# cxy1997/3D_adapt_auto_driving

Hardware: AMD Instinct MI355X
Metric: KITTI scenes/s end-to-end eval_rcnn (joint RPN+RCNN, synthetic 16384-pt scenes) (higher is better)
Workload: dtype f32; 1 GPU; BASELINE.json configs[2]: full PointRCNN RPN+RCNN inference, default.yaml shapes, random-init weights, batch=8 synthetic KITTI scenes x 16384 pts per GPU per step; scene=synth.scenes (SURVEY 8d: uniform clutter + ground + 10 dense cars), parallelism=scene-sharded x1, one final all_gather of detections, detections_gathered=652455, batch_slots=14, look_ahead=12, steps_per_launch=2

## Files before the change

3d_adapt_auto_driving_amd/csrc/fps.hip:

```cpp
#include "common.hpp"
#include <math.h>
#include <stdlib.h>
#include <map>
#include <mutex>

namespace prcnn {

__device__ __forceinline__ bool better(float v, uint32_t key, float bv, uint32_t bkey)
{
    return (v > bv) | ((v == bv) & (key < bkey));
}

__device__ __forceinline__ void take_if_better(float v, uint32_t key, float &bv, uint32_t &bkey)
{
    const bool t = better(v, key, bv, bkey);
    bv = t ? v : bv;
    bkey = t ? key : bkey;
}

template <int CTRL>
__device__ __forceinline__ int dpp_mov(int x)
{
    return __builtin_amdgcn_update_dpp(x, x, CTRL, 0xf, 0xf, false);
}
// ... 42 lines not shown
    else r = fmax_raw(v, __int_as_float(dpp_mov<CTRL>(__float_as_int(v))));
    return r;
}
template <int CTRL>
__device__ __forceinline__ uint32_t dpp_min(uint32_t v)
{
    uint32_t r;
    if constexpr (CTRL == 0xB1) PRCNN_DPP_OP("v_min_u32_dpp", uint32_t, "quad_perm:[1,0,3,2]");
    else if constexpr (CTRL == 0x4E) PRCNN_DPP_OP("v_min_u32_dpp", uint32_t, "quad_perm:[2,3,0,1]");
    else if constexpr (CTRL == 0x141) PRCNN_DPP_OP("v_min_u32_dpp", uint32_t, "row_half_mirror");
    else if constexpr (CTRL == 0x140) PRCNN_DPP_OP("v_min_u32_dpp", uint32_t, "row_mirror");
    else {
        const uint32_t o = (uint32_t)dpp_mov<CTRL>((int)v);
        r = o < v ? o : v;
    }
    return r;
}
__device__ __forceinline__ float wave_max_f32(float v)
{
    v = dpp_max<0xB1>(v); v = dpp_max<0x4E>(v); v = dpp_max<0x141>(v); v = dpp_max<0x140>(v);
    const float r0 = __int_as_float(__builtin_amdgcn_readlane(__float_as_int(v), 0));
    const float r1 = __int_as_float(__builtin_amdgcn_readlane(__float_as_int(v), 16));
    const float r2 = __int_as_float(__builtin_amdgcn_readlane(__float_as_int(v), 32));
    const float r3 = __int_as_float(__builtin_amdgcn_readlane(__float_as_int(v), 48));
    return fmaxf(fmaxf(r0, r1), fmaxf(r2, r3));
}
__device__ __forceinline__ uint32_t wave_min_u32(uint32_t v)
{
    v = dpp_min<0xB1>(v); v = dpp_min<0x4E>(v); v = dpp_min<0x141>(v); v = dpp_min<0x140>(v);
    const uint32_t r0 = (uint32_t)__builtin_amdgcn_readlane((int)v, 0), r1 = (uint32_t)__builtin_amdgcn_readlane((int)v, 16);
    const uint32_t r2 = (uint32_t)__builtin_amdgcn_readlane((int)v, 32), r3 = (uint32_t)__builtin_amdgcn_readlane((int)v, 48);
    const uint32_t a = r0 < r1 ? r0 : r1, b = r2 < r3 ? r2 : r3;
    return a < b ? a : b;
}
__device__ __forceinline__ unsigned long long pack_candidate(float v, uint32_t key)
{
    const uint32_t b = (uint32_t)__float_as_int(v);
    const uint32_t mono = (b & 0x80000000u) ? ~b : (b | 0x80000000u);
    return ((unsigned long long)mono << 32) | (unsigned long long)(~key);
}
__device__ __forceinline__ void unpack_candidate(unsigned long long w, float &v, uint32_t &key)
{
    const uint32_t mono = (uint32_t)(w >> 32);
    const uint32_t b = (mono & 0x80000000u) ? (mono & 0x7fffffffu) : ~mono;
    v = __int_as_float((int)b);
    key = ~(uint32_t)w;
}

template <bool HIPCC>
__device__ __forceinline__ float fps_dist(float px, float py, float pz, float ox, float oy, float oz)
{
    if (!HIPCC) return sqdist3(px, py, pz, ox, oy, oz);
    const float dx = px - ox, dy = py - oy, dz = pz - oz;
    return __fadd_rn(__fmaf_rn(dy, dy, __fmul_rn(dx, dx)), __fmul_rn(dz, dz));
}

struct KeyCodec {
    int log2bs;
    int sh;
    int hipcc;
    __device__ __forceinline__ uint32_t encode(int k) const
    {
        const uint32_t low = (uint32_t)k & ((1u << log2bs) - 1u);
        const uint32_t rev = log2bs ? (__brev(low) >> (32 - log2bs)) : 0u;
        return (rev << sh) | ((uint32_t)k >> log2bs);
    }
    __device__ __forceinline__ int decode(uint32_t key) const
    {
        const uint32_t hi = key >> sh;
        const uint32_t rev = log2bs ? (__brev(hi) >> (32 - log2bs)) : 0u;
        return (int)(((key & ((1u << sh) - 1u)) << log2bs) | rev);
    }
};

template <int WAVES, int PPT, bool ORDERED>
__global__ __launch_bounds__(64 * WAVES) void fps_reg_kernel(
    int n, int m, KeyCodec kc, const float *__restrict__ xyz, float *__restrict__ temp,
    int *__restrict__ idx, float *__restrict__ new_xyz = nullptr, const int *__restrict__ rejected = nullptr)
{
    constexpr int T = 64 * WAVES;
    __shared__ unsigned long long s_best[3];
    const int b = blockIdx.x;
    if (rejected && rejected[b] == 0) return;
    const float *__restrict__ cloud = xyz + (long)b * n * 3;
    float *__restrict__ mind = temp ? temp + (long)b * n : nullptr;
    int *__restrict__ sel = idx + (long)b * m;
    float *__restrict__ nxyz = new_xyz ? new_xyz + (long)b * m * 3 : nullptr;
    const int t = threadIdx.x;
    __builtin_amdgcn_s_setprio(3);

    float px[PPT], py[PPT], pz[PPT], pt[PPT];
    uint32_t pk[PPT];
#pragma unroll
    for (int i = 0; i < PPT; ++i) {
        const int k = t + i * T;
        if (k < n) {
            px[i] = cloud[3 * k]; py[i] = cloud[3 * k + 1]; pz[i] = cloud[3 * k + 2];
            pt[i] = mind ? mind[k] : 1e10f;
            pk[i] = kc.encode(k);
        } else {
            px[i] = py[i] = pz[i] = 0.f;
            pt[i] = -INFINITY;
            pk[i] = 0xffffffffu;
        }
    }
    if (WAVES > 1 && t < 3) s_best[t] = 0ull;
    if (WAVES > 1) __syncthreads();

    int old = 0;
    if (t == 0) sel[0] = 0;
    for (int j = 1; j < m; ++j) {
        float ox, oy, oz;
        if constexpr (WAVES == 1) {
            const int pl = old & 63, pi = old >> 6;
            ox = oy = oz = 0.f;
#pragma unroll
            for (int i = 0; i < PPT; ++i) {
                const float vx = __int_as_float(__builtin_amdgcn_readlane(__float_as_int(px[i]), pl));
                const float vy = __int_as_float(__builtin_amdgcn_readlane(__float_as_int(py[i]), pl));
                const float vz = __int_as_float(__builtin_amdgcn_readlane(__float_as_int(pz[i]), pl));
                if (i == pi) { ox = vx; oy = vy; oz = vz; }
            }
        } else {
            ox = cloud[3 * old]; oy = cloud[3 * old + 1]; oz = cloud[3 * old + 2];
        }
        if (nxyz && t == 0) { nxyz[3 * (j - 1)] = ox; nxyz[3 * (j - 1) + 1] = oy; nxyz[3 * (j - 1) + 2] = oz; }
        float lv = -INFINITY;
        if (kc.hipcc) {
#pragma unroll
            for (int i = 0; i < PPT; ++i) {
                const float d2 = fminf(fps_dist<true>(px[i], py[i], pz[i], ox, oy, oz), pt[i]);
                pt[i] = d2;
                lv = fmaxf(lv, d2);
            }
        } else {
#pragma unroll
            for (int i = 0; i < PPT; ++i) {
                const float d = sqdist3(px[i], py[i], pz[i], ox, oy, oz);
                const float d2 = fminf(d, pt[i]);
                pt[i] = d2;
                lv = fmaxf(lv, d2);
            }
        }
        float bv = wave_max_f32(lv);
        uint32_t lk = 0xffffffffu;
#pragma unroll
        for (int i = 0; i < PPT; ++i) {
            const uint32_t c = pt[i] == bv ? pk[i] : 0xffffffffu;
            lk = c < lk ? c : lk;
        }
        uint32_t bkey = wave_min_u32(lk);
        if (WAVES > 1) {
            const int buf = j % 3;
            if ((t & 63) == 0) atomicMax(&s_best[buf], pack_candidate(bv, bkey));
            lds_barrier();
            const unsigned long long best = s_best[buf];
            if (t == 0) s_best[(j + 2) % 3] = 0ull;
            unpack_candidate(best, bv, bkey);
        }
        old = (bkey == 0xffffffffu || !(bv > -1.0f)) ? 0 : kc.decode(bkey);
        old = __builtin_amdgcn_readfirstlane(old);
        if (t == 0) sel[j] = old;
        if (bv == 0.f) {
            for (int jj = j + 1 + t; jj < m; jj += T) {
                sel[jj] = 0;
                if (nxyz) { nxyz[3 * (jj - 1)] = cloud[0]; nxyz[3 * (jj - 1) + 1] = cloud[1]; nxyz[3 * (jj - 1) + 2] = cloud[2]; }
            }
            if (nxyz && t == 0) { nxyz[3 * j] = cloud[0]; nxyz[3 * j + 1] = cloud[1]; nxyz[3 * j + 2] = cloud[2]; }
            break;
        }
    }
    if (nxyz && t == 0 && m > 0) { nxyz[3 * (m - 1)] = cloud[3 * old]; nxyz[3 * (m - 1) + 1] = cloud[3 * old + 1]; nxyz[3 * (m - 1) + 2] = cloud[3 * old + 2]; }
    if (mind) {
#pragma unroll
        for (int i = 0; i < PPT; ++i) {
            const int k = t + i * T;
            if (k < n) mind[k] = pt[i];
        }
    }
}


__device__ __forceinline__ unsigned part1by1(unsigned v)
{
    v &= 0xffffu;
    v = (v | (v << 8)) & 0x00ff00ffu;
    v = (v | (v << 4)) & 0x0f0f0f0fu;
    v = (v | (v << 2)) & 0x33333333u;
    v = (v | (v << 1)) & 0x55555555u;
    return v;
}

__global__ __launch_bounds__(1024) void fps_order_kernel(int n, const float *__restrict__ xyz, int *__restrict__ perm,
                                                         const int *__restrict__ rejected = nullptr)
// ... 79 lines not shown
    if (rejected && rejected[b] == 0) return;
    const float *__restrict__ cloud = xyz + (long)b * n * 3;
    const int *__restrict__ order = perm + (long)b * n;
    float *__restrict__ mind = temp ? temp + (long)b * n : nullptr;
    int *__restrict__ sel = idx + (long)b * m;
    float *__restrict__ nxyz = new_xyz ? new_xyz + (long)b * m * 3 : nullptr;
    const int t = threadIdx.x, lane = t & 63, w = t >> 6;
    __builtin_amdgcn_s_setprio(3);

    float px[PPT], py[PPT], pz[PPT], pt[PPT];
    uint32_t pc[PPT];
    float bx0 = INFINITY, bx1 = -INFINITY, by0 = INFINITY, by1 = -INFINITY, bz0 = INFINITY, bz1 = -INFINITY;
#pragma unroll
    for (int i = 0; i < PPT; ++i) {
        const int s = w * (64 * PPT) + i * 64 + lane;
        float x0 = INFINITY, x1 = -INFINITY, y0 = INFINITY, y1 = -INFINITY, z0 = INFINITY, z1 = -INFINITY;
        if (s < n) {
            const int k = order[s];
            px[i] = cloud[3 * k]; py[i] = cloud[3 * k + 1]; pz[i] = cloud[3 * k + 2];
            pt[i] = mind ? mind[k] : 1e10f;
            pc[i] = (kc.encode(k) << SB) | (uint32_t)i;
            x0 = x1 = px[i]; y0 = y1 = py[i]; z0 = z1 = pz[i];
        } else {
            px[i] = py[i] = pz[i] = 0.f;
            pt[i] = -INFINITY;
            pc[i] = 0xffffffffu;
        }
#pragma unroll
        for (int d = 32; d >= 1; d >>= 1) {
            x0 = fmin_raw(x0, __shfl_xor(x0, d, 64)); x1 = fmax_raw(x1, __shfl_xor(x1, d, 64));
            y0 = fmin_raw(y0, __shfl_xor(y0, d, 64)); y1 = fmax_raw(y1, __shfl_xor(y1, d, 64));
            z0 = fmin_raw(z0, __shfl_xor(z0, d, 64)); z1 = fmax_raw(z1, __shfl_xor(z1, d, 64));
        }
        if (lane == i) { bx0 = x0; bx1 = x1; by0 = y0; by1 = y1; bz0 = z0; bz1 = z1; }
    }

    constexpr int GP = 64 / PPT;
    bx0 = __shfl(bx0, lane & (PPT - 1), 64); bx1 = __shfl(bx1, lane & (PPT - 1), 64);
    by0 = __shfl(by0, lane & (PPT - 1), 64); by1 = __shfl(by1, lane & (PPT - 1), 64);
    bz0 = __shfl(bz0, lane & (PPT - 1), 64); bz1 = __shfl(bz1, lane & (PPT - 1), 64);
    unsigned long long touched = 0ull, etiles = ~0ull;
    float bound = INFINITY;
    auto box_mask = [&](float ox, float oy, float oz, bool live) __attribute__((always_inline)) {
        const float dx = fmax_raw(fmax_raw(bx0 - ox, ox - bx1), 0.f);
        const float dy = fmax_raw(fmax_raw(by0 - oy, oy - by1), 0.f);
        const float dz = fmax_raw(fmax_raw(bz0 - oz, oz - bz1), 0.f);
        const float lb = dx * dx + dy * dy + dz * dz;
        return __ballot(live && !(lb * 0.99999f >= bound));
    };
    auto update = [&](float ox, float oy, float oz, unsigned long long mask) __attribute__((always_inline)) {
        if (mask != 0ull) {
            touched |= mask & etiles;
            const pk_f32x2 o_x = {ox, ox}, o_y = {oy, oy}, o_z = {oz, oz};
            if (kc.hipcc) {
#pragma unroll
                for (int i = 0; i < PPT; i += 2)
                    if ((mask >> i) & 3ull) {
                        const pk_f32x2 dx = (pk_f32x2){px[i], px[i + 1]} - o_x, dy = (pk_f32x2){py[i], py[i + 1]} - o_y,
                                       dz = (pk_f32x2){pz[i], pz[i + 1]} - o_z;
                        const pk_f32x2 d = __builtin_elementwise_fma(dy, dy, dx * dx) + dz * dz;
                        pt[i] = fmin_raw(d.x, pt[i]); pt[i + 1] = fmin_raw(d.y, pt[i + 1]);
                    }
            } else {
#pragma unroll
                for (int i = 0; i < PPT; i += 2)
                    if ((mask >> i) & 3ull) {
                        const pk_f32x2 dx = (pk_f32x2){px[i], px[i + 1]} - o_x, dy = (pk_f32x2){py[i], py[i + 1]} - o_y,
                                       dz = (pk_f32x2){pz[i], pz[i + 1]} - o_z;
                        const pk_f32x2 d = (dx * dx + dy * dy) + dz * dz;
                        pt[i] = fmin_raw(d.x, pt[i]); pt[i + 1] = fmin_raw(d.y, pt[i + 1]);
                    }
            }
        }
    };
    if (t == 0) {
        sel[0] = 0;
        if (nxyz) { nxyz[0] = cloud[0]; nxyz[1] = cloud[1]; nxyz[2] = cloud[2]; }
    }
    if (t < 32) { s_rank[t] = 0; s_blk[t] = 0; }
    int j = 1;
    if (m > 1) {
        const float ox = cloud[0], oy = cloud[1], oz = cloud[2];
        update(ox, oy, oz, box_mask(ox, oy, oz, lane < PPT));
    }
    touched = ~0ull;
    while (j < m) {
        if (touched != 0ull) {
            float bv = -INFINITY, sv = -INFINITY;
#pragma unroll
            for (int i = 0; i < PPT; ++i) {
                sv = __builtin_amdgcn_fmed3f(bv, sv, pt[i]);
                bv = fmax_raw(bv, pt[i]);
            }
            uint32_t lk = 0xffffffffu;
#pragma unroll
            for (int i = 0; i < PPT; ++i) {
                const uint32_t c = pt[i] == bv ? pc[i] : 0xffffffffu;
                lk = c < lk ? c : lk;
            }
            const float v1 = wave_max_f32(bv);
            const uint32_t c1 = wave_min_u32(bv == v1 ? lk : 0xffffffffu);
            const unsigned long long m1 = __ballot(bv == v1 && lk == c1);
            const int l1 = m1 ? (int)__builtin_ctzll(m1) : 0;
            const float bv2 = lane == l1 ? -INFINITY : bv;
            const float v2 = wave_max_f32(bv2);
            const uint32_t c2 = wave_min_u32(bv2 == v2 ? lk : 0xffffffffu);
            const unsigned long long m2 = __ballot(lane != l1 && bv2 == v2 && lk == c2);
            const int l2 = m2 ? (int)__builtin_ctzll(m2) : l1;
            const float v3 = wave_max_f32((lane == l1 || lane == l2) ? -INFINITY : bv);
            const float s1 = __int_as_float(__builtin_amdgcn_readlane(__float_as_int(sv), l1));
            const float s2 = __int_as_float(__builtin_amdgcn_readlane(__float_as_int(sv), l2));
            const float wB = fmax_raw(v3, fmax_raw(s1, s2));
            bound = v1;
            const int sl1 = (int)(c1 & ((1u << SB) - 1u)), sl2 = (int)(c2 & ((1u << SB) - 1u));
            const bool has2 = m2 != 0ull && c2 != 0xffffffffu;
            etiles = (1ull << sl1) | (has2 ? (1ull << sl2) : 0ull);
            float x1 = 0.f, y1 = 0.f, z1 = 0.f, x2 = 0.f, y2 = 0.f, z2 = 0.f;
            fs_pick3<PPT>(px, py, pz, __builtin_amdgcn_readfirstlane(sl1), l1, x1, y1, z1);
            fs_pick3<PPT>(px, py, pz, __builtin_amdgcn_readfirstlane(sl2), l2, x2, y2, z2);
            const float ex = lane == 0 ? x1 : x2, ey = lane == 0 ? y1 : y2, ez = lane == 0 ? z1 : z2;
            if (lane < 2) {
                const float ev = lane == 0 ? v1 : (has2 ? v2 : -INFINITY);
                const uint32_t ek = lane == 0 ? (c1 == 0xffffffffu ? 0xffffffffu : (c1 >> SB)) : (has2 ? (c2 >> SB) : 0xffffffffu);
                s_vk[2 * w + lane] = pack_candidate(ev, ek);
                s_xyz[2 * w + lane][0] = ex; s_xyz[2 * w + lane][1] = ey; s_xyz[2 * w + lane][2] = ez;
                if (lane == 0) s_bound[w] = wB;
            }
        }
        lds_barrier();
        const int left = m - j;
        const int e = lane & 31, h = lane >> 5;
        const unsigned long long pke = s_vk[e];
        float cv; uint32_t ck;
        unpack_candidate(pke, cv, ck);
        const float cx = s_xyz[e][0], cy = s_xyz[e][1], cz = s_xyz[e][2];
        const float gB = wave_max_f32(lane < 16 ? s_bound[lane] : -INFINITY);
        {
            const int i = 2 * w + h;
            const unsigned long long pki = s_vk[i];
            float iv; uint32_t ik;
            unpack_candidate(pki, iv, ik);
            const float ix = s_xyz[i][0], iy = s_xyz[i][1], iz = s_xyz[i][2];
            const bool before = pke > pki;
            const float d = kc.hipcc ? fps_dist<true>(ix, iy, iz, cx, cy, cz) : sqdist3(ix, iy, iz, cx, cy, cz);
            const unsigned long long bb = __ballot(before), kb = __ballot(before && (d < iv));
            if (e == 0) {
                s_rank[i] = __popc((unsigned)(h ? (bb >> 32) : bb));
                s_blk[i] = (unsigned)(h ? (kb >> 32) : kb) != 0u;
            }
        }
        lds_barrier();
        const int rank = s_rank[e];
        const bool blocked = s_blk[e] != 0;
        const bool valid = !(ck == 0xffffffffu || !(cv > -1.0f));
        const bool pass = rank == 0 ? true : ((cv > gB) && (cv > 0.f) && valid && !blocked);
        const bool stop = !pass || (rank == 0 && !valid);
        int r = (int)wave_min_u32((stop && !(rank == 0)) ? (uint32_t)rank : ((rank == 0 && !valid) ? 1u : 32u));
        r = min(min(r, left), FS_RMAX);
        if (r < 1) r = 1;
        const float ox_ = valid ? cx : cloud[0], oy_ = valid ? cy : cloud[1], oz_ = valid ? cz : cloud[2];
        if (w == 0 && h == 0 && rank < r) {
            sel[j + rank] = valid ? kc.decode(ck) : 0;
            if (nxyz) { nxyz[3 * (j + rank)] = ox_; nxyz[3 * (j + rank) + 1] = oy_; nxyz[3 * (j + rank) + 2] = oz_; }
        }
        const int dst = (h == 0 && rank < FS_RMAX) ? 3 * rank : 63;
        const float rv = __int_as_float(__builtin_amdgcn_ds_permute(dst << 2, __float_as_int(ox_)) |
                                        __builtin_amdgcn_ds_permute(min(dst + 1, 63) << 2, __float_as_int(oy_)) |
                                        __builtin_amdgcn_ds_permute(min(dst + 2, 63) << 2, __float_as_int(oz_)));
        j += r;
        const int apply_n = j >= m ? r - 1 : r;
        touched = 0ull;
        for (int q0 = 0; q0 < apply_n; q0 += GP) {
            const int qg = q0 + lane / PPT;
            const int src = 3 * min(qg, FS_RMAX - 1);
            const float gx = __shfl(rv, src, 64), gy = __shfl(rv, src + 1, 64), gz = __shfl(rv, src + 2, 64);
            const unsigned long long masks = box_mask(gx, gy, gz, qg < apply_n);
            if (masks == 0ull) continue;
#pragma unroll
            for (int g = 0; g < GP; ++g) {
                const unsigned long long mk = (masks >> (g * PPT)) & ((PPT == 64) ? ~0ull : ((1ull << PPT) - 1ull));
                if (mk != 0ull) {
                    const int q = q0 + g;
                    const float ox = __int_as_float(__builtin_amdgcn_readlane(__float_as_int(rv), 3 * q));
                    const float oy = __int_as_float(__builtin_amdgcn_readlane(__float_as_int(rv), 3 * q + 1));
                    const float oz = __int_as_float(__builtin_amdgcn_readlane(__float_as_int(rv), 3 * q + 2));
                    update(ox, oy, oz, mk);
                }
            }
        }
    }
    if (mind) {
#pragma unroll
        for (int i = 0; i < PPT; ++i)
            if (pc[i] != 0xffffffffu) mind[kc.decode(pc[i] >> SB)] = pt[i];
    }
}

struct Fps2Table {
    unsigned long long vk[2][64];
    float xyz[2][64][4];
    float bound[2][32];
    unsigned int sync;
    unsigned int pad[63];
};

__device__ __forceinline__ unsigned long long ld_agent_u64(const unsigned long long *p)
{
    return __hip_atomic_load(p, __ATOMIC_RELAXED, __HIP_MEMORY_SCOPE_AGENT);
}
__device__ __forceinline__ float ld_agent_f32(const float *p)
{
    return __int_as_float(__hip_atomic_load(reinterpret_cast<const int *>(p), __ATOMIC_RELAXED, __HIP_MEMORY_SCOPE_AGENT));
}

__device__ __forceinline__ void st_agent_u64(unsigned long long *p, unsigned long long v)
{
    __hip_atomic_store(p, v, __ATOMIC_RELAXED, __HIP_MEMORY_SCOPE_AGENT);
}
__device__ __forceinline__ void st_agent_f32(float *p, float v)
{
    __hip_atomic_store(reinterpret_cast<int *>(p), __float_as_int(v), __ATOMIC_RELAXED, __HIP_MEMORY_SCOPE_AGENT);
}

__global__ __launch_bounds__(1024) void fps_spec2_kernel(
    int nclouds, int n, int m, KeyCodec kc, const float *__restrict__ xyz, const int *__restrict__ perm,
    float *__restrict__ temp, int *__restrict__ idx, float *__restrict__ new_xyz, Fps2Table *__restrict__ tables)
{
    constexpr int PPT = 16, SB = 4, NE = 64;
    __shared__ unsigned long long s_vk[NE];
    __shared__ float s_xyz[NE][3];
    __shared__ float s_bound[32];
    __shared__ float s_res[64];
    __shared__ int s_rank[NE], s_blk[NE];
    __shared__ unsigned long long s_evk[32];
    __shared__ float s_exyz[32][3], s_eb[16];
    const int q_ = blockIdx.x;
    const int b = (q_ >> 4) * 8 + (q_ & 7), half = (q_ >> 3) & 1;
    if (b >= nclouds) return;
    const float *__restrict__ cloud = xyz + (long)b * n * 3;
    const int *__restrict__ order = perm + (long)b * n;
    float *__restrict__ mind = temp ? temp + (long)b * n : nullptr;
    int *__restrict__ sel = idx + (long)b * m;
    float *__restrict__ nxyz = new_xyz ? new_xyz + (long)b * m * 3 : nullptr;
    Fps2Table *__restrict__ tb = tables + b;
    const int t = threadIdx.x, lane = t & 63, w = t >> 6, gw = 16 * half + w;
    __builtin_amdgcn_s_setprio(3);

    float px[PPT], py[PPT], pz[PPT], pt[PPT];
    uint32_t pc[PPT];
    float bx0 = INFINITY, bx1 = -INFINITY, by0 = INFINITY, by1 = -INFINITY, bz0 = INFINITY, bz1 = -INFINITY;
#pragma unroll
// ... 414 lines not shown
    else if (n <= 16384) launch_reg<16, 16>(b, n, m, kc, xyz, temp, idx, st, nullptr, rejected);
    else hipLaunchKernelGGL(fps_generic_kernel, dim3(b), dim3(1024), 0, st, n, m, kc, xyz, temp, idx);
    return check_launch("furthest_point_sampling");
}

extern "C" int prcnn_furthest_point_sampling(int b, int n, int m, const float *xyz, float *temp,
                                             int *idx, void *stream)
{
    PRCNN_REQUIRE(temp || b == 0 || m == 0, "fps: null pointer");
    return fps_any(b, n, m, xyz, temp, idx, nullptr, stream);
}

static int fps_new_xyz_any(int b, int n, int m, const float *xyz, int *idx, float *new_xyz, void *stream, const int *rejected)
{
    if (n > 1024) return fps_any(b, n, m, xyz, nullptr, idx, new_xyz, stream, rejected);
    hipStream_t st = (hipStream_t)stream;
    KeyCodec kc;
    if (const int rc = fps_codec(n, &kc)) return rc;
    if (n <= 128) launch_reg<1, 2>(b, n, m, kc, xyz, nullptr, idx, st, new_xyz, rejected);
    else if (n <= 256) launch_reg<1, 4>(b, n, m, kc, xyz, nullptr, idx, st, new_xyz, rejected);
    else if (n <= 512) launch_reg<1, 8>(b, n, m, kc, xyz, nullptr, idx, st, new_xyz, rejected);
    else if (b >= 128) launch_reg<1, 16>(b, n, m, kc, xyz, nullptr, idx, st, new_xyz, rejected);
    else launch_reg<4, 4>(b, n, m, kc, xyz, nullptr, idx, st, new_xyz, rejected);
    return check_launch("fps_new_xyz");
}

extern "C" int prcnn_fps_new_xyz(int b, int n, int m, const float *xyz, int *idx, float *new_xyz, void *stream)
{
    PRCNN_REQUIRE(b >= 0 && n > 0 && m >= 0, "fps_new_xyz: b=%d n=%d m=%d", b, n, m);
    if (b == 0 || m == 0) return PRCNN_OK;
    PRCNN_REQUIRE(xyz && idx && new_xyz, "fps_new_xyz: null pointer");
    return fps_new_xyz_any(b, n, m, xyz, idx, new_xyz, stream, nullptr);
}

namespace prcnn {
constexpr int FPX_T = 256;

template <bool HIPCC>
__global__ __launch_bounds__(FPX_T) void fps_prefix_pivots_kernel(int n, int m, const float *__restrict__ xyz, float *__restrict__ dpiv,
                                                                  int *__restrict__ rejected, int *__restrict__ idx, float *__restrict__ new_xyz)
{
    __shared__ float s_p[FPX_T][3];
    __shared__ float s_part[4][64];
    const int b = blockIdx.y, t = threadIdx.x, lane = t & 63, w = t >> 6;
    const float *__restrict__ cloud = xyz + (long)b * n * 3;
    if (blockIdx.x == 0 && t == 0) rejected[b] = 0;
    const int s = blockIdx.x * 64 + lane;
    const int sc = min(s, m - 1);
    const float x = cloud[3 * sc], y = cloud[3 * sc + 1], z = cloud[3 * sc + 2];
    const int iend = min(blockIdx.x * 64 + 63, m - 1);
    float d = 1e10f;
    for (int i0 = 0; i0 < iend; i0 += FPX_T) {
        __syncthreads();
        if (i0 + t < iend) { s_p[t][0] = cloud[3 * (i0 + t)]; s_p[t][1] = cloud[3 * (i0 + t) + 1]; s_p[t][2] = cloud[3 * (i0 + t) + 2]; }
        __syncthreads();
        const int k1 = min(64, iend - i0 - 64 * w);
#pragma unroll 4
        for (int k = 0; k < k1; ++k) {
            const int q = 64 * w + k;
            const float e = fps_dist<HIPCC>(x, y, z, s_p[q][0], s_p[q][1], s_p[q][2]);
            d = (i0 + q < s) ? fminf(e, d) : d;
        }
    }
    s_part[w][lane] = d;
    __syncthreads();
    if (w == 0 && s < m) {
        dpiv[(long)b * m + s] = fminf(fminf(s_part[0][lane], s_part[1][lane]), fminf(s_part[2][lane], s_part[3][lane]));
        if (idx) idx[(long)b * m + s] = s;
        if (new_xyz) { float *o = new_xyz + ((long)b * m + s) * 3; o[0] = x; o[1] = y; o[2] = z; }
    }
}

template <bool HIPCC>
__global__ __launch_bounds__(FPX_T) void fps_prefix_check_kernel(int n, int m, KeyCodec kc, const float *__restrict__ xyz,
                                                                 const float *__restrict__ dpiv, int *__restrict__ rejected)
{
    __shared__ float4 s_p[FPX_T];
    const int b = blockIdx.y, t = threadIdx.x;
    const float *__restrict__ cloud = xyz + (long)b * n * 3;
    const float *__restrict__ D = dpiv + (long)b * m;
    const int j = blockIdx.x * FPX_T + t, jc = min(j, n - 1);
    const float x = cloud[3 * jc], y = cloud[3 * jc + 1], z = cloud[3 * jc + 2];
    const uint32_t kj = kc.encode(jc);
    bool ok = fabsf(x) < INFINITY && fabsf(y) < INFINITY && fabsf(z) < INFINITY;
    if (jc >= 1 && jc < m) ok &= D[jc] > 0.f;
    const int jmax = min(n, (int)(blockIdx.x + 1) * FPX_T) - 1;
    const int iend = min(m, jmax) - 1;
    float r = 1e10f;
    for (int i0 = 0; ; i0 += FPX_T) {
        const int seen = __hip_atomic_load(rejected + b, __ATOMIC_RELAXED, __HIP_MEMORY_SCOPE_AGENT);
        if (__syncthreads_or(!ok || seen != 0) || i0 >= iend) break;
        if (i0 + t < iend) {
            const int i = i0 + t;
            s_p[t] = make_float4(cloud[3 * i], cloud[3 * i + 1], cloud[3 * i + 2], D[i + 1]);
        }
        __syncthreads();
        const int k1 = min(FPX_T, iend - i0);
#pragma unroll 4
        for (int k = 0; k < k1; ++k) {
            const float4 p = s_p[k];
            const int s = i0 + k + 1;
            r = fminf(fps_dist<HIPCC>(x, y, z, p.x, p.y, p.z), r);
            bool win = p.w > r;
            if (p.w == r) win = kc.encode(s) < kj;
            ok = ok && (win || s >= jc);
        }
    }
    if (!ok) rejected[b] = 1;
}
}

extern "C" int prcnn_fps_nested_supported(int n, int m) { return m >= 2 && m <= n && n <= 16384; }

static int fps_prefix_any(int b, int n, int m, const KeyCodec &kc, const float *xyz, int *idx, float *new_xyz, float *dpiv, int *rejected,
                          hipStream_t st)
{
    const dim3 g1((unsigned)((m + 63) / 64), (unsigned)b), g2((unsigned)((n + FPX_T - 1) / FPX_T), (unsigned)b);
    if (kc.hipcc) {
        hipLaunchKernelGGL(fps_prefix_pivots_kernel<true>, g1, dim3(FPX_T), 0, st, n, m, xyz, dpiv, rejected, idx, new_xyz);
        hipLaunchKernelGGL(fps_prefix_check_kernel<true>, g2, dim3(FPX_T), 0, st, n, m, kc, xyz, dpiv, rejected);
    } else {
        hipLaunchKernelGGL(fps_prefix_pivots_kernel<false>, g1, dim3(FPX_T), 0, st, n, m, xyz, dpiv, rejected, idx, new_xyz);
        hipLaunchKernelGGL(fps_prefix_check_kernel<false>, g2, dim3(FPX_T), 0, st, n, m, kc, xyz, dpiv, rejected);
    }
    return check_launch("fps_prefix_check");
}

extern "C" int prcnn_fps_prefix_check(int b, int n, int m, const float *xyz, int *idx, float *new_xyz, int *rejected, void *stream)
{
    PRCNN_REQUIRE(b >= 0 && b <= 65535 && prcnn_fps_nested_supported(n, m), "fps_prefix_check: b=%d n=%d m=%d", b, n, m);
    if (b == 0) return PRCNN_OK;
    PRCNN_REQUIRE(xyz && rejected, "fps_prefix_check: null pointer");
    hipStream_t st = (hipStream_t)stream;
    KeyCodec kc;
    if (const int rc = fps_codec(n, &kc)) return rc;
    float *dpiv = (float *)scratch_for(st, (size_t)b * m * sizeof(float), 15);
    if (!dpiv) { set_error("fps_prefix_check: cannot allocate the pivot scratch"); return PRCNN_ELAUNCH; }
    return fps_prefix_any(b, n, m, kc, xyz, idx, new_xyz, dpiv, rejected, st);
}

extern "C" int prcnn_fps_new_xyz_flagged(int b, int n, int m, const float *xyz, int *idx, float *new_xyz, const int *rejected, void *stream)
{
    PRCNN_REQUIRE(b >= 0 && prcnn_fps_nested_supported(n, m), "fps_new_xyz_flagged: b=%d n=%d m=%d", b, n, m);
    if (b == 0) return PRCNN_OK;
    PRCNN_REQUIRE(xyz && idx && new_xyz && rejected, "fps_new_xyz_flagged: null pointer");
    return fps_new_xyz_any(b, n, m, xyz, idx, new_xyz, stream, rejected);
}

extern "C" int prcnn_fps_new_xyz_nested(int b, int n, int m, const float *xyz, int *idx, float *new_xyz, void *stream)
{
    PRCNN_REQUIRE(b >= 0 && n > 0 && m >= 0, "fps_new_xyz_nested: b=%d n=%d m=%d", b, n, m);
    if (b == 0 || m == 0) return PRCNN_OK;
    PRCNN_REQUIRE(xyz && idx && new_xyz, "fps_new_xyz_nested: null pointer");
    if (!prcnn_fps_nested_supported(n, m) || b > 65535) return fps_new_xyz_any(b, n, m, xyz, idx, new_xyz, stream, nullptr);
    hipStream_t st = (hipStream_t)stream;
    KeyCodec kc;
    if (const int rc = fps_codec(n, &kc)) return rc;
    float *dpiv = (float *)scratch_for(st, ((size_t)b * m + (size_t)b) * sizeof(float), 15);
    if (!dpiv) { set_error("fps_new_xyz_nested: cannot allocate the check's scratch"); return PRCNN_ELAUNCH; }
    int *rejected = (int *)(dpiv + (size_t)b * m);
    if (const int rc = fps_prefix_any(b, n, m, kc, xyz, idx, new_xyz, dpiv, rejected, st)) return rc;
    return fps_new_xyz_any(b, n, m, xyz, idx, new_xyz, stream, rejected);
}
namespace prcnn {
__global__ __launch_bounds__(256) void point_groups_kernel(int n, const float *__restrict__ xyz, const int *__restrict__ perm,
                                                           float4 *__restrict__ pxyz, float4 *__restrict__ aabb)
{
    const int b = blockIdx.y, lane = threadIdx.x & 63;
    const int g = blockIdx.x * 4 + (threadIdx.x >> 6);
    if (g * 64 >= n) return;
    const long s = (long)b * n + g * 64 + lane;
    const int k = perm[s];
    const float *p = xyz + ((long)b * n + k) * 3;
    const float x = p[0], y = p[1], z = p[2];
    pxyz[s] = make_float4(x, y, z, __int_as_float(k));
    float x0 = x, x1 = x, y0 = y, y1 = y, z0 = z, z1 = z;
#pragma unroll
    for (int d = 32; d >= 1; d >>= 1) {
        x0 = fminf(x0, __shfl_xor(x0, d, 64)); x1 = fmaxf(x1, __shfl_xor(x1, d, 64));
        y0 = fminf(y0, __shfl_xor(y0, d, 64)); y1 = fmaxf(y1, __shfl_xor(y1, d, 64));
        z0 = fminf(z0, __shfl_xor(z0, d, 64)); z1 = fmaxf(z1, __shfl_xor(z1, d, 64));
    }
    if (lane == 0) {
        aabb[((long)b * (n / 64) + g) * 2] = make_float4(x0, y0, z0, 0.f);
        aabb[((long)b * (n / 64) + g) * 2 + 1] = make_float4(x1, y1, z1, 0.f);
    }
}
}

extern "C" int prcnn_point_groups(int b, int n, const float *xyz, float *pxyz, float *aabb, void *stream)
{
    PRCNN_REQUIRE(b >= 0 && n > 0 && n % 64 == 0 && n <= 65536 && b <= 65535, "point_groups: b=%d n=%d (n a multiple of 64, <= 65536)", b, n);
    if (b == 0) return PRCNN_OK;
    PRCNN_REQUIRE(xyz && pxyz && aabb && (((uintptr_t)pxyz | (uintptr_t)aabb) & 15) == 0, "point_groups: null / misaligned pointer");
    hipStream_t st = (hipStream_t)stream;
    int *perm = (int *)scratch_for(st, (size_t)b * n * sizeof(int), 8);
    if (!perm) { set_error("point_groups: cannot allocate ordering scratch"); return PRCNN_ELAUNCH; }
    hipLaunchKernelGGL(fps_order_kernel, dim3(b), dim3(1024), 0, st, n, xyz, perm);
    hipLaunchKernelGGL(point_groups_kernel, dim3((n / 64 + 3) / 4, b), dim3(256), 0, st, n, xyz, perm, (float4 *)pxyz, (float4 *)aabb);
    return check_launch("point_groups");
}

namespace prcnn {

constexpr int RG_N = 512, RG_M1 = 128, RG_M2 = 32, RG_NS = 64;
constexpr int RG_LD1 = RG_M1 + 1, RG_LD2 = RG_M2 + 1;

template <int PPT, int D, int I = 0>
__device__ __forceinline__ void roi_pick3(const float (&px)[PPT], const float (&py)[PPT], const float (&pz)[PPT], int slot, int l,
                                          float &x, float &y, float &z)
{
    if (I + 1 == D || slot == I) {
        x = __int_as_float(__builtin_amdgcn_readlane(__float_as_int(px[I]), l));
        y = __int_as_float(__builtin_amdgcn_readlane(__float_as_int(py[I]), l));
        z = __int_as_float(__builtin_amdgcn_readlane(__float_as_int(pz[I]), l));
    } else if constexpr (I + 1 < D) {
        roi_pick3<PPT, D, I + 1>(px, py, pz, slot, l, x, y, z);
    }
}

template <int PPT, int D, bool MOD>
// ... 402 lines not shown
```

profiles/fps_round_sim.py:

```python
import os, sys, importlib, numpy as np
sys.path.insert(0, os.path.dirname(os.path.dirname(os.path.abspath(__file__))))
S = importlib.import_module('3d_adapt_auto_driving_amd.synth')

def morton_order(p):
    x, z = p[:, 0], p[:, 2]
    gx = np.clip(((x - x.min()) / max(x.max() - x.min(), 1e-9) * 64).astype(int), 0, 63)
    gz = np.clip(((z - z.min()) / max(z.max() - z.min(), 1e-9) * 64).astype(int), 0, 63)
    def part(v):
        v = v.astype(np.uint32); r = np.zeros_like(v)
        for b in range(6): r |= ((v >> b) & 1) << (2 * b)
        return r
    code = part(gx) | (part(gz) << 1)
    return np.argsort(code, kind='stable')

def simulate(p, m, layout, PPT=16, top=2, rmax=16, stats=None, W=16, greedy=False):
    n = p.shape[0]
    order = morton_order(p)
    w_, i_, l_ = np.meshgrid(np.arange(W), np.arange(PPT), np.arange(64), indexing='ij')
    if layout == 'blocked':
        s = w_ * 64 * PPT + i_ * 64 + l_
    elif layout == 'interleaved':
        s = (i_ * W + w_) * 64 + l_
    elif layout == 'quad':
        g, wi = w_ // 4, w_ % 4
        s = g * (4 * 64 * PPT) + (i_ * 4 + wi) * 64 + l_
    idx = order[s]
    P = p[idx].astype(np.float32)
    pt = np.full((W, PPT, 64), 1e10, np.float32)
    def upd(o):
        d = ((P - o) ** 2).sum(-1).astype(np.float32)
        np.minimum(pt, d, out=pt)
    upd(p[0].astype(np.float32))
    j, rounds = 1, 0
    hist = np.zeros(rmax + 1, int)
    why = {'bound': 0, 'blocked': 0, 'rmax': 0, 'end': 0}
    while j < m:
        lane_best = pt.max(1)
        lane_arg = pt.argmax(1)
        srt = np.sort(pt, axis=1)
        lane_second = srt[:, -2, :]
        ordl = np.argsort(-lane_best, axis=1, kind='stable')
        ents = []
        wB = np.zeros(W, np.float32)
        for w in range(W):
            ls = ordl[w, :top]
            third = lane_best[w, ordl[w, top]]
            wB[w] = max(third, lane_second[w, ls].max())
            for l in ls:
                ents.append((lane_best[w, l], idx[w, lane_arg[w, l], l], w))
        ents.sort(key=lambda e: (-e[0], e[1]))
        gB = wB.max()
        if greedy:
            E = np.array([p[e[1]] for e in ents], np.float32)
            val = np.array([e[0] for e in ents], np.float32)
            key = np.array([e[1] for e in ents])
            alive = np.ones(len(ents), bool)
            acc, reason = [], 'rmax'
            while True:
                if len(acc) >= min(rmax, m - j): reason = 'rmax' if len(acc) >= rmax else 'end'; break
                cand = np.where(alive)[0]
                if len(cand) == 0: reason = 'entries'; break
                b = cand[np.lexsort((key[cand], -val[cand]))[0]]
                if acc and not (val[b] > gB): reason = 'bound'; break
                acc.append(ents[b]); alive[b] = False
                d = ((E - E[b]) ** 2).sum(-1).astype(np.float32)
                val = np.minimum(val, d)
            why[reason] = why.get(reason, 0) + 1
            hist[len(acc)] += 1
            for a in acc: upd(p[a[1]].astype(np.float32))
            j += len(acc); rounds += 1
            continue
        acc = [ents[0]]
        reason = 'rmax'
        for e in ents[1:]:
            if len(acc) >= min(rmax, m - j): reason = 'rmax' if len(acc) >= rmax else 'end'; break
            if not (e[0] > gB): reason = 'bound'; break
            pe = p[e[1]].astype(np.float32)
            blk = False
            for a in ents:
                if a is e: break
                if ((p[a[1]].astype(np.float32) - pe) ** 2).sum() < e[0]: blk = True; break
            if blk: reason = 'blocked'; break
            acc.append(e)
        else:
            reason = 'rmax'
        why[reason] += 1
        hist[len(acc)] += 1
        for a in acc: upd(p[a[1]].astype(np.float32))
        j += len(acc); rounds += 1
    return rounds, hist, why

def simulate_lazy(p, m, mode, PPT=16, W=16, rmax=16):
    order = morton_order(p)
    w_, i_, l_ = np.meshgrid(np.arange(W), np.arange(PPT), np.arange(64), indexing='ij')
    idx = order[w_ * 64 * PPT + i_ * 64 + l_]
    P = p[idx].astype(np.float32)
    lo, hi = P.min(2), P.max(2)
    pt = np.full((W, PPT, 64), 1e10, np.float32)
    np.minimum(pt, ((P - p[0].astype(np.float32)) ** 2).sum(-1).astype(np.float32), out=pt)
    cache = [None] * W
    bound = np.full(W, np.inf, np.float32)
    j = 1; rounds = 0; rebuilds = 0; touched_tot = 0
    def build(w):
        lane_best = pt[w].max(0); lane_arg = pt[w].argmax(0)
        lane_second = np.sort(pt[w], axis=0)[-2]
        ordl = np.argsort(-lane_best, kind='stable')
        ls = ordl[:2]
        wB = max(lane_best[ordl[2]], lane_second[ls].max())
        return [(lane_best[l], idx[w, lane_arg[l], l], w, (lane_arg[l], l)) for l in ls], wB, lane_best[ordl[0]]
    need = np.ones(W, bool)
    while j < m:
        for w in range(W):
            if need[w]:
                cache[w] = build(w); rebuilds += 1; bound[w] = cache[w][2]
        ents = sorted((e for w in range(W) for e in cache[w][0]), key=lambda e: (-e[0], e[1]))
        gB = max(c[1] for c in cache)
        acc = [ents[0]]
        for e in ents[1:]:
            if len(acc) >= min(rmax, m - j) or not (e[0] > gB): break
            pe = p[e[1]].astype(np.float32)
            blk = False
            for a in ents:
                if a is e: break
                if ((p[a[1]].astype(np.float32) - pe) ** 2).sum() < e[0]: blk = True; break
            if blk: break
            acc.append(e)
        old = pt.copy()
        touched = np.zeros(W, bool); tt = np.zeros((W, PPT), bool)
        for a in acc:
            o = p[a[1]].astype(np.float32)
            d = np.maximum(np.maximum(lo - o, o - hi), 0)
            tmask = (d * d).sum(-1) * 0.99999 < bound[:, None]
            touched |= tmask.any(1); tt |= tmask
            dd = ((P - o) ** 2).sum(-1).astype(np.float32)
            np.minimum(pt, np.where(tmask[:, :, None], dd, pt), out=pt)
        touched_tot += touched.sum()
        if mode == 'E':
            need = np.array([any(pt[w][e[3]] < old[w][e[3]] for e in cache[w][0]) for w in range(W)])
        elif mode == 'Etile':
            need = np.array([any(tt[w, e[3][0]] for e in cache[w][0]) for w in range(W)])
        else:
            need = touched
        j += len(acc); rounds += 1
    return rounds, rebuilds / rounds, touched_tot / rounds


if __name__ == '__main__':
    kind = sys.argv[1]; m = int(sys.argv[2]) if len(sys.argv) > 2 else 4096
    make = S.lidar_scenes if kind == 'lidar' else S.scenes
    pts = make(2, 16384, seed0=0)
    if len(sys.argv) > 3 and sys.argv[3] == 'lazy':
        for mode in ('touched', 'E', 'Etile'):
            r, rb, tc = simulate_lazy(pts[0][:, :3], m, mode)
            print(kind, mode, 'rounds', r, 'rebuilds per round %.2f' % rb, 'box-touched waves per round %.2f' % tc, flush=True)
        sys.exit(0)
    if len(sys.argv) > 3 and sys.argv[3] == 'greedy':
        for g in (False, True):
            r, h, why = simulate(pts[0][:, :3], m, 'blocked', top=2, greedy=g)
            print(kind, 'blocked', 'greedy' if g else 'prefix', 'rounds', r, 'picks/round %.2f' % ((m - 1) / r), why, 'hist', h.tolist(), flush=True)
        sys.exit(0)
    for layout in ('blocked', 'quad', 'interleaved'):
        for top in (2,):
            r, h, why = simulate(pts[0][:, :3], m, layout, top=top)
            print(kind, layout, 'top', top, 'rounds', r, 'picks/round %.2f' % ((m - 1) / r), why, 'hist', h.tolist(), flush=True)
```

Baseline: 8880 scenes/s.

## Resume FPS fallback from first failing prefix pick and extend batched rounds greedily

```diff
diff --git a/3d_adapt_auto_driving_amd/csrc/fps.hip b/3d_adapt_auto_driving_amd/csrc/fps.hip
--- a/3d_adapt_auto_driving_amd/csrc/fps.hip
+++ b/3d_adapt_auto_driving_amd/csrc/fps.hip
@@ -148,6 +148,7 @@
     __shared__ unsigned long long s_best[3];
     const int b = blockIdx.x;
     if (rejected && rejected[b] == 0) return;
+    const int first = rejected ? min(max(rejected[b], 1), max(m - 1, 1)) : 1;
     const float *__restrict__ cloud = xyz + (long)b * n * 3;
     float *__restrict__ mind = temp ? temp + (long)b * n : nullptr;
     int *__restrict__ sel = idx + (long)b * m;
@@ -173,9 +174,24 @@
     if (WAVES > 1 && t < 3) s_best[t] = 0ull;
     if (WAVES > 1) __syncthreads();
 
-    int old = 0;
+    int old = first - 1;
     if (t == 0) sel[0] = 0;
-    for (int j = 1; j < m; ++j) {
+    if (first > 1) {
+        for (int s = 1 + t; s < first; s += T) {
+            sel[s] = s;
+            if (nxyz) { nxyz[3 * (s - 1)] = cloud[3 * (s - 1)]; nxyz[3 * (s - 1) + 1] = cloud[3 * (s - 1) + 1]; nxyz[3 * (s - 1) + 2] = cloud[3 * (s - 1) + 2]; }
+        }
+#pragma unroll 4
+        for (int s = 0; s < first - 1; ++s) {
+            const float ox = cloud[3 * s], oy = cloud[3 * s + 1], oz = cloud[3 * s + 2];
+#pragma unroll
+            for (int i = 0; i < PPT; ++i) {
+                const float d = kc.hipcc ? fps_dist<true>(px[i], py[i], pz[i], ox, oy, oz) : sqdist3(px[i], py[i], pz[i], ox, oy, oz);
+                pt[i] = fminf(d, pt[i]);
+            }
+        }
+    }
+    for (int j = first; j < m; ++j) {
         float ox, oy, oz;
         if constexpr (WAVES == 1) {
             const int pl = old & 63, pi = old >> 6;
@@ -421,6 +437,26 @@
     if (m > 1) {
         const float ox = cloud[0], oy = cloud[1], oz = cloud[2];
         update(ox, oy, oz, box_mask(ox, oy, oz, lane < PPT));
+    }
+    if (rejected) {
+        const int first = min(max(rejected[b], 1), max(m - 1, 1));
+        for (int s = 1 + t; s < first; s += 1024) {
+            sel[s] = s;
+            if (nxyz) { nxyz[3 * s] = cloud[3 * s]; nxyz[3 * s + 1] = cloud[3 * s + 1]; nxyz[3 * s + 2] = cloud[3 * s + 2]; }
+        }
+#pragma nounroll
+        for (int s = 1; s < first; ++s) {
+            const float ox = cloud[3 * s], oy = cloud[3 * s + 1], oz = cloud[3 * s + 2];
+            const pk_f32x2 o_x = {ox, ox}, o_y = {oy, oy}, o_z = {oz, oz};
+#pragma unroll
+            for (int i = 0; i < PPT; i += 2) {
+                const pk_f32x2 dx = (pk_f32x2){px[i], px[i + 1]} - o_x, dy = (pk_f32x2){py[i], py[i + 1]} - o_y,
+                               dz = (pk_f32x2){pz[i], pz[i + 1]} - o_z;
+                const pk_f32x2 d = kc.hipcc ? __builtin_elementwise_fma(dy, dy, dx * dx) + dz * dz : (dx * dx + dy * dy) + dz * dz;
+                pt[i] = fmin_raw(d.x, pt[i]); pt[i + 1] = fmin_raw(d.y, pt[i + 1]);
+            }
+        }
+        j = first;
     }
     touched = ~0ull;
     while (j < m) {
@@ -495,7 +531,9 @@
         const bool pass = rank == 0 ? true : ((cv > gB) && (cv > 0.f) && valid && !blocked);
         const bool stop = !pass || (rank == 0 && !valid);
         int r = (int)wave_min_u32((stop && !(rank == 0)) ? (uint32_t)rank : ((rank == 0 && !valid) ? 1u : 32u));
-        r = min(min(r, left), FS_RMAX);
+        const bool go_on = __ballot(h == 0 && rank == r && rank != 0 && (cv > gB) && (cv > 0.f) && valid) != 0ull;
+        const int rcap = min(left, FS_RMAX);
+        r = min(r, rcap);
         if (r < 1) r = 1;
         const float ox_ = valid ? cx : cloud[0], oy_ = valid ? cy : cloud[1], oz_ = valid ? cz : cloud[2];
         if (w == 0 && h == 0 && rank < r) {
@@ -503,9 +541,38 @@
             if (nxyz) { nxyz[3 * (j + rank)] = ox_; nxyz[3 * (j + rank) + 1] = oy_; nxyz[3 * (j + rank) + 2] = oz_; }
         }
         const int dst = (h == 0 && rank < FS_RMAX) ? 3 * rank : 63;
-        const float rv = __int_as_float(__builtin_amdgcn_ds_permute(dst << 2, __float_as_int(ox_)) |
-                                        __builtin_amdgcn_ds_permute(min(dst + 1, 63) << 2, __float_as_int(oy_)) |
-                                        __builtin_amdgcn_ds_permute(min(dst + 2, 63) << 2, __float_as_int(oz_)));
+        float rv = __int_as_float(__builtin_amdgcn_ds_permute(dst << 2, __float_as_int(ox_)) |
+                                  __builtin_amdgcn_ds_permute(min(dst + 1, 63) << 2, __float_as_int(oy_)) |
+                                  __builtin_amdgcn_ds_permute(min(dst + 2, 63) << 2, __float_as_int(oz_)));
+        if (go_on && r < rcap) {
+            auto edist = [&](float qx, float qy, float qz) __attribute__((always_inline)) {
+                return kc.hipcc ? fps_dist<true>(cx, cy, cz, qx, qy, qz) : sqdist3(cx, cy, cz, qx, qy, qz);
+            };
+            float val = (h == 0 && rank >= r && valid) ? cv : -INFINITY;
+            for (int q = 0; q < r; ++q) {
+                const float qx = __int_as_float(__builtin_amdgcn_readlane(__float_as_int(rv), 3 * q));
+                const float qy = __int_as_float(__builtin_amdgcn_readlane(__float_as_int(rv), 3 * q + 1));
+                const float qz = __int_as_float(__builtin_amdgcn_readlane(__float_as_int(rv), 3 * q + 2));
+                val = fmin_raw(edist(qx, qy, qz), val);
+            }
+            while (r < rcap) {
+                const float bv = wave_max_f32(val);
+                if (!(bv > gB) || !(bv > 0.f)) break;
+                const uint32_t bk = wave_min_u32(val == bv ? ck : 0xffffffffu);
+                const unsigned long long mb = __ballot(val == bv && ck == bk);
+                const int l = (int)__builtin_ctzll(mb);
+                const float qx = __int_as_float(__builtin_amdgcn_readlane(__float_as_int(cx), l));
+                const float qy = __int_as_float(__builtin_amdgcn_readlane(__float_as_int(cy), l));
+                const float qz = __int_as_float(__builtin_amdgcn_readlane(__float_as_int(cz), l));
+                if (t == 0) {
+                    sel[j + r] = kc.decode(bk);
+                    if (nxyz) { nxyz[3 * (j + r)] = qx; nxyz[3 * (j + r) + 1] = qy; nxyz[3 * (j + r) + 2] = qz; }
+                }
+                rv = lane == 3 * r ? qx : (lane == 3 * r + 1 ? qy : (lane == 3 * r + 2 ? qz : rv));
+                val = lane == l ? -INFINITY : fmin_raw(edist(qx, qy, qz), val);
+                ++r;
+            }
+        }
         j += r;
         const int apply_n = j >= m ? r - 1 : r;
         touched = 0ull;
@@ -1086,14 +1153,24 @@
     const int j = blockIdx.x * FPX_T + t, jc = min(j, n - 1);
     const float x = cloud[3 * jc], y = cloud[3 * jc + 1], z = cloud[3 * jc + 2];
     const uint32_t kj = kc.encode(jc);
-    bool ok = fabsf(x) < INFINITY && fabsf(y) < INFINITY && fabsf(z) < INFINITY;
-    if (jc >= 1 && jc < m) ok &= D[jc] > 0.f;
+    int fs = (fabsf(x) < INFINITY && fabsf(y) < INFINITY && fabsf(z) < INFINITY) ? 0 : 1;
+    if (fs == 0 && jc >= 1 && jc < m && !(D[jc] > 0.f)) fs = jc;
+    int told = 0;
+    auto report = [&]() __attribute__((always_inline)) {
+        if (fs != told) {
+            int cur = __hip_atomic_load(rejected + b, __ATOMIC_RELAXED, __HIP_MEMORY_SCOPE_AGENT);
+            while ((cur == 0 || cur > fs) &&
+                   !__hip_atomic_compare_exchange_strong(rejected + b, &cur, fs, __ATOMIC_RELAXED, __ATOMIC_RELAXED, __HIP_MEMORY_SCOPE_AGENT)) {}
+            told = fs;
+        }
+    };
     const int jmax = min(n, (int)(blockIdx.x + 1) * FPX_T) - 1;
     const int iend = min(m, jmax) - 1;
     float r = 1e10f;
     for (int i0 = 0; ; i0 += FPX_T) {
+        report();
         const int seen = __hip_atomic_load(rejected + b, __ATOMIC_RELAXED, __HIP_MEMORY_SCOPE_AGENT);
-        if (__syncthreads_or(!ok || seen != 0) || i0 >= iend) break;
+        if (__syncthreads_or(seen != 0 && seen <= i0) || i0 >= iend) break;
         if (i0 + t < iend) {
             const int i = i0 + t;
             s_p[t] = make_float4(cloud[3 * i], cloud[3 * i + 1], cloud[3 * i + 2], D[i + 1]);
@@ -1107,10 +1184,15 @@
             r = fminf(fps_dist<HIPCC>(x, y, z, p.x, p.y, p.z), r);
             bool win = p.w > r;
             if (p.w == r) win = kc.encode(s) < kj;
-            ok = ok && (win || s >= jc);
-        }
-    }
-    if (!ok) rejected[b] = 1;
+            fs = (fs == 0 && !(win || s >= jc)) ? s : fs;
+        }
+    }
+    report();
+}
+__global__ __launch_bounds__(256) void fps_prefix_flag_kernel(int b, const int *__restrict__ first, int *__restrict__ rejected)
+{
+    const int i = blockIdx.x * 256 + threadIdx.x;
+    if (i < b) rejected[i] = first[i] != 0;
 }
 }
 
@@ -1138,9 +1220,12 @@
     hipStream_t st = (hipStream_t)stream;
     KeyCodec kc;
     if (const int rc = fps_codec(n, &kc)) return rc;
-    float *dpiv = (float *)scratch_for(st, (size_t)b * m * sizeof(float), 15);
+    float *dpiv = (float *)scratch_for(st, ((size_t)b * m + (size_t)b) * sizeof(float), 15);
     if (!dpiv) { set_error("fps_prefix_check: cannot allocate the pivot scratch"); return PRCNN_ELAUNCH; }
-    return fps_prefix_any(b, n, m, kc, xyz, idx, new_xyz, dpiv, rejected, st);
+    int *first = (int *)(dpiv + (size_t)b * m);
+    if (const int rc = fps_prefix_any(b, n, m, kc, xyz, idx, new_xyz, dpiv, first, st)) return rc;
+    hipLaunchKernelGGL(fps_prefix_flag_kernel, dim3((unsigned)((b + 255) / 256)), dim3(256), 0, st, b, first, rejected);
+    return check_launch("fps_prefix_check(flags)");
 }
 
 extern "C" int prcnn_fps_new_xyz_flagged(int b, int n, int m, const float *xyz, int *idx, float *new_xyz, const int *rejected, void *stream)
diff --git a/profiles/fps_round_sim.py b/profiles/fps_round_sim.py
--- a/profiles/fps_round_sim.py
+++ b/profiles/fps_round_sim.py
@@ -90,7 +90,7 @@
         j += len(acc); rounds += 1
     return rounds, hist, why
 
-def simulate_lazy(p, m, mode, PPT=16, W=16, rmax=16):
+def simulate_lazy(p, m, mode, PPT=16, W=16, rmax=16, greedy=False):
     order = morton_order(p)
     w_, i_, l_ = np.meshgrid(np.arange(W), np.arange(PPT), np.arange(64), indexing='ij')
     idx = order[w_ * 64 * PPT + i_ * 64 + l_]
@@ -100,7 +100,7 @@
     np.minimum(pt, ((P - p[0].astype(np.float32)) ** 2).sum(-1).astype(np.float32), out=pt)
     cache = [None] * W
     bound = np.full(W, np.inf, np.float32)
-    j = 1; rounds = 0; rebuilds = 0; touched_tot = 0
+    j = 1; rounds = 0; rebuilds = 0; touched_tot = 0; greedy_picks = [0]
     def build(w):
         lane_best = pt[w].max(0); lane_arg = pt[w].argmax(0)
         lane_second = np.sort(pt[w], axis=0)[-2]
@@ -116,6 +116,7 @@
         ents = sorted((e for w in range(W) for e in cache[w][0]), key=lambda e: (-e[0], e[1]))
         gB = max(c[1] for c in cache)
         acc = [ents[0]]
+        go_on = False
         for e in ents[1:]:
             if len(acc) >= min(rmax, m - j) or not (e[0] > gB): break
             pe = p[e[1]].astype(np.float32)
@@ -123,8 +124,18 @@
             for a in ents:
                 if a is e: break
                 if ((p[a[1]].astype(np.float32) - pe) ** 2).sum() < e[0]: blk = True; break
-            if blk: break
+            if blk: go_on = greedy and e[0] > 0; break
             acc.append(e)
+        if go_on:
+            rest = ents[len(acc):]
+            E = np.array([p[e[1]] for e in rest], np.float32)
+            val = np.array([e[0] for e in rest], np.float32); key = np.array([e[1] for e in rest])
+            for a in acc: val = np.minimum(val, ((E - p[a[1]].astype(np.float32)) ** 2).sum(-1).astype(np.float32))
+            while len(acc) < min(rmax, m - j):
+                b = np.lexsort((key, -val))[0]
+                if not (val[b] > gB and val[b] > 0): break
+                acc.append(rest[b]); greedy_picks[0] += 1
+                val = np.minimum(val, ((E - E[b]) ** 2).sum(-1).astype(np.float32)); val[b] = -np.inf
         old = pt.copy()
         touched = np.zeros(W, bool); tt = np.zeros((W, PPT), bool)
         for a in acc:
@@ -142,6 +153,7 @@
         else:
             need = touched
         j += len(acc); rounds += 1
+    if greedy: print('    picks made behind a blocked entry: %d of %d' % (greedy_picks[0], m - 1))
     return rounds, rebuilds / rounds, touched_tot / rounds
 
 
@@ -158,6 +170,9 @@
         for g in (False, True):
             r, h, why = simulate(pts[0][:, :3], m, 'blocked', top=2, greedy=g)
             print(kind, 'blocked', 'greedy' if g else 'prefix', 'rounds', r, 'picks/round %.2f' % ((m - 1) / r), why, 'hist', h.tolist(), flush=True)
+        for g in (False, True):
+            r, rb, tc = simulate_lazy(pts[0][:, :3], m, 'Etile', greedy=g)
+            print(kind, 'Etile', 'greedy' if g else 'prefix', 'rounds', r, 'rebuilds per round %.2f' % rb, flush=True)
         sys.exit(0)
     for layout in ('blocked', 'quad', 'interleaved'):
         for top in (2,):
```

After: 8705 scenes/s. 2.0% lower.
